# Apokleos/kata-xpu-device-plugin

Measured on NVIDIA H100. Metric: pci.ids parse GB/s (x1000 text + 2^20-key join); device lookups/s reported beside it, higher is better.
Workload: dtype u8

## Files before the change

kata-xpu-device-plugin_b200/csrc/parse_common.cuh:

```cuda
#pragma once
#include "common.cuh"
#include "table.cuh"

namespace kxparse {

constexpr int CW = 2048;
constexpr int HALF = 1024;
constexpr int TRAIL = 16;
constexpr int STG_BYTES = CW + TRAIL;
constexpr int WARPS = 8;
constexpr int NT = WARPS * 32;

constexpr unsigned long long ST_NONE = 1ull << 62;
constexpr unsigned long long ST_PREFIX = 2ull << 62;
constexpr unsigned long long ST_MASK = 3ull << 62;
constexpr unsigned long long CV_HAS_TOP = 1ull << 61;
constexpr unsigned long long CV_VOK = 1ull << 60;
constexpr unsigned long long CV_ANCHOR_MASK = (1ull << 44) - 1;
constexpr uint32_t KX_MAX_PROBE = 1024;
constexpr uint32_t P_NONE = 0xFFFFFFFFu;
#define LS_PUB 0x80000000u
#define LS_TOP 0x40000000u
#define LS_VOK 0x20000000u

__device__ __forceinline__ uint32_t smem_u32(const void *p) { return (uint32_t)__cvta_generic_to_shared(p); }
__device__ __forceinline__ void mbar_init(unsigned long long *bar, uint32_t count) {
    asm volatile("mbarrier.init.shared::cta.b64 [%0], %1;" ::"r"(smem_u32(bar)), "r"(count));
}

__device__ __forceinline__ unsigned long long l2_evict_first_policy() {
    unsigned long long pol;
    asm volatile("createpolicy.fractional.L2::evict_first.b64 %0, 1.0;" : "=l"(pol));
    return pol;
}

__device__ __forceinline__ uint32_t lop3_and_xor(uint32_t a, uint32_t b, uint32_t c) {
    uint32_t d;
    asm("lop3.b32 %0, %1, %2, %3, 0x6A;" : "=r"(d) : "r"(a), "r"(b), "r"(c));
    return d;
}
__device__ __forceinline__ uint32_t lop3_nor_and(uint32_t a, uint32_t b, uint32_t c) {
    uint32_t d;
    asm("lop3.b32 %0, %1, %2, %3, 0x02;" : "=r"(d) : "r"(a), "r"(b), "r"(c));
    return d;
}

__device__ __forceinline__ uint32_t nl_mask16(const uint4 v, uint32_t k7f, uint32_t k0a, uint32_t k80) {
    uint32_t f0 = lop3_nor_and(lop3_and_xor(v.x, k7f, k0a) + k7f, v.x, k80);
    uint32_t f1 = lop3_nor_and(lop3_and_xor(v.y, k7f, k0a) + k7f, v.y, k80);
    uint32_t f2 = lop3_nor_and(lop3_and_xor(v.z, k7f, k0a) + k7f, v.z, k80);
    uint32_t f3 = lop3_nor_and(lop3_and_xor(v.w, k7f, k0a) + k7f, v.w, k80);
    uint32_t lo = __dp4a(f0, 0x08040201u, 0u);
    lo = __dp4a(f1, 0x80402010u, lo);
    uint32_t hi = __dp4a(f2, 0x08040201u, 0u);
    hi = __dp4a(f3, 0x80402010u, hi);
    return (lo >> 7) | (hi << 1);
}

__device__ __forceinline__ bool hex4_swar(uint32_t x, uint32_t &val) {
    uint32_t v = (x & 0x0f0f0f0fu) + ((x >> 6) & 0x01010101u) * 9u;
    uint32_t r = v + 0x30303030u + (((v + 0x06060606u) >> 4) & 0x01010101u) * 0x27u;
    uint32_t s = __byte_perm(v, 0u, 0x0123);
    uint32_t u = s | (s >> 4);
    val = __byte_perm(u, 0u, 0x4420);
    return ((v & 0xf0f0f0f0u) == 0u) & (r == x);
}

__device__ __forceinline__ void table_fold(const KxTableDev &tb, uint32_t key, unsigned long long line_g,
                                           unsigned long long anchor_g, uint32_t &fresh_cnt) {
    uint32_t slot = key == KX_EMPTY_KEY ? tb.cap : (kx_hash(key) >> tb.shift);
    uint4 head = __ldcg(reinterpret_cast<const uint4 *>(&tb.slots[slot]));
    uint32_t k = head.x;
    unsigned long long ml = ((unsigned long long)head.w << 32) | head.z;
    if (key != KX_EMPTY_KEY && k != key) {
        uint32_t step = 0;
        bool fresh = false;
        for (;;) {
            if (k == KX_EMPTY_KEY) {
                uint32_t old = atomicCAS(&tb.slots[slot].key, KX_EMPTY_KEY, key);
                if (old == KX_EMPTY_KEY) {
                    fresh_cnt++;
                    fresh = true;
                    break;
                }
                if (old == key) break;
            }
            slot = (slot + 1) & (tb.cap - 1);
            if (++step >= KX_MAX_PROBE) { tb.counters[KX_C_OVERFLOW] = 1u; return; }
            k = __ldcg(&tb.slots[slot].key);
            if (k == key) break;
        }
        ml = fresh ? KX_NO_OFF : __ldcg(&tb.slots[slot].min_line);
    }
    if (line_g < ml) {
        atomicMin(&tb.slots[slot].min_line, line_g);
        atomicMin(&tb.slots[slot].min_anchor, anchor_g);
    }
}

__device__ __forceinline__ void table_fold_claim2(const KxTableDev &tb, uint32_t key0, unsigned long long line0, unsigned long long anchor0,
                                                  bool on1, uint32_t key1, unsigned long long line1, unsigned long long anchor1,
                                                  uint32_t &fresh_cnt) {
    uint32_t slot0 = key0 == KX_EMPTY_KEY ? tb.cap : (kx_hash(key0) >> tb.shift);
    uint32_t slot1 = key1 == KX_EMPTY_KEY ? tb.cap : (kx_hash(key1) >> tb.shift);
    bool open0 = key0 != KX_EMPTY_KEY, open1 = on1 && key1 != KX_EMPTY_KEY, ok0 = true, ok1 = on1;
    for (uint32_t step = 0; open0 || open1; step++) {
        uint32_t old0 = 0, old1 = 0;
        if (open0) old0 = atomicCAS(&tb.slots[slot0].key, KX_EMPTY_KEY, key0);
        if (open1) old1 = atomicCAS(&tb.slots[slot1].key, KX_EMPTY_KEY, key1);
        if (open0) {
            if (old0 == KX_EMPTY_KEY) { fresh_cnt++; open0 = false; }
            else if (old0 == key0) open0 = false;
            else slot0 = (slot0 + 1) & (tb.cap - 1);
        }
        if (open1) {
            if (old1 == KX_EMPTY_KEY) { fresh_cnt++; open1 = false; }
            else if (old1 == key1) open1 = false;
            else slot1 = (slot1 + 1) & (tb.cap - 1);
        }
        if (step + 1 >= KX_MAX_PROBE && (open0 || open1)) {
            tb.counters[KX_C_OVERFLOW] = 1u;
            ok0 = ok0 && !open0; ok1 = ok1 && !open1;
            break;
        }
    }
    if (ok0) { atomicMin(&tb.slots[slot0].min_line, line0); atomicMin(&tb.slots[slot0].min_anchor, anchor0); }
    if (ok1) { atomicMin(&tb.slots[slot1].min_line, line1); atomicMin(&tb.slots[slot1].min_anchor, anchor1); }
}

__device__ __forceinline__ int32_t table_probe(const KxSlot *__restrict__ slots, uint32_t cap, uint32_t shift, uint32_t key) {
    if (key == KX_EMPTY_KEY) return slots[cap].row;
    uint32_t slot = kx_hash(key) >> shift;
    for (uint32_t step = 0; step < cap; step++) {
        const uint2 kr = __ldg(reinterpret_cast<const uint2 *>(&slots[slot]));
        if (kr.x == key) return (int32_t)kr.y;
        if (kr.x == KX_EMPTY_KEY) return -1;
        slot = (slot + 1) & (cap - 1);
    }
    return -1;
}

__device__ __forceinline__ void table_probe4(const KxSlot *__restrict__ slots, uint32_t cap, uint32_t shift, const uint32_t (&key)[4],
                                             uint32_t on, int32_t (&row)[4]) {
    uint32_t slot[4], open = on & 0xfu;
#pragma unroll
    for (int j = 0; j < 4; j++) {
        row[j] = -1;
        slot[j] = key[j] == KX_EMPTY_KEY ? cap : (kx_hash(key[j]) >> shift);
    }
    for (uint32_t step = 0; open && step < cap; step++) {
        uint2 kr[4];
#pragma unroll
        for (int j = 0; j < 4; j++)
            if ((open >> j) & 1u) kr[j] = __ldg(reinterpret_cast<const uint2 *>(&slots[slot[j]]));
#pragma unroll
        for (int j = 0; j < 4; j++) {
            if (!((open >> j) & 1u)) continue;
            if (slot[j] == cap || kr[j].x == key[j]) { row[j] = (int32_t)kr[j].y; open &= ~(1u << j); }
            else if (kr[j].x == KX_EMPTY_KEY) open &= ~(1u << j);
            else slot[j] = (slot[j] + 1) & (cap - 1);
        }
    }
}

__device__ __forceinline__ uint32_t table_claim(const KxTableDev &tb, uint32_t key, uint32_t &fresh_cnt) {
    if (key == KX_EMPTY_KEY) return tb.cap;
    uint32_t slot = kx_hash(key) >> tb.shift;
    for (uint32_t step = 0; step < KX_MAX_PROBE; step++) {
        const uint32_t k = __ldcg(&tb.slots[slot].key);
        if (k == key) return slot;
        if (k == KX_EMPTY_KEY) {
            const uint32_t old = atomicCAS(&tb.slots[slot].key, KX_EMPTY_KEY, key);
            if (old == KX_EMPTY_KEY) { fresh_cnt++; return slot; }
            if (old == key) return slot;
        }
        slot = (slot + 1) & (tb.cap - 1);
    }
    tb.counters[KX_C_OVERFLOW] = 1u;
    return 0xffffffffu;
}

__device__ __forceinline__ uint32_t table_find(const KxTableDev &tb, uint32_t key) {
    if (key == KX_EMPTY_KEY) return tb.cap;
    uint32_t slot = kx_hash(key) >> tb.shift;
    for (uint32_t step = 0; step < tb.cap; step++) {
        const uint32_t k = __ldg(&tb.slots[slot].key);
        if (k == key) return slot;
        if (k == KX_EMPTY_KEY) return 0xffffffffu;
        slot = (slot + 1) & (tb.cap - 1);
    }
    return 0xffffffffu;
}

__device__ __forceinline__ uint4 lds128(uint32_t a) {
    uint4 v;
    asm volatile("ld.shared.v4.u32 {%0, %1, %2, %3}, [%4];" : "=r"(v.x), "=r"(v.y), "=r"(v.z), "=r"(v.w) : "r"(a));
    return v;
}
__device__ __forceinline__ uint32_t lds32(uint32_t a) {
    uint32_t v;
    asm volatile("ld.shared.u32 %0, [%1];" : "=r"(v) : "r"(a));
    return v;
}
__device__ __forceinline__ uint32_t lds8(uint32_t a) {
    uint32_t v;
    asm volatile("ld.shared.u8 %0, [%1];" : "=r"(v) : "r"(a));
    return v;
}
__device__ __forceinline__ uint32_t lds32_unaligned(uint32_t a) {
    const uint32_t al = a & ~3u;
    return __funnelshift_r(lds32(al), lds32(al + 4u), (a & 3u) * 8u);
}
__device__ __forceinline__ void mbar_expect_tx_a(uint32_t bar, uint32_t bytes) {
    asm volatile("mbarrier.arrive.expect_tx.shared::cta.b64 _, [%0], %1;" ::"r"(bar), "r"(bytes) : "memory");
}
__device__ __forceinline__ bool mbar_try_a(uint32_t bar, uint32_t parity) {
    uint32_t ok;
    asm volatile("{ .reg .pred p; mbarrier.try_wait.parity.shared::cta.b64 p, [%1], %2; selp.u32 %0, 1, 0, p; }"
                 : "=r"(ok)
                 : "r"(bar), "r"(parity)
                 : "memory");
    return ok != 0u;
}
__device__ __forceinline__ void tma_load_a(uint32_t dst, const void *src, uint32_t bytes, uint32_t bar, unsigned long long pol) {
    asm volatile("cp.async.bulk.shared::cluster.global.mbarrier::complete_tx::bytes.L2::cache_hint [%0], [%1], %2, [%3], %4;" ::"r"(dst),
                 "l"(src), "r"(bytes), "r"(bar), "l"(pol)
                 : "memory");
}

__device__ __forceinline__ uint32_t stage_chunk_manual(const uint8_t *text, unsigned long long n, uint32_t g, uint32_t lane,
                                                       uint8_t *dst) {
    const unsigned long long chunk_start = (unsigned long long)g * CW;
    const unsigned long long remain = n - chunk_start;
    const uint32_t n_rel = remain < (unsigned long long)CW ? (uint32_t)remain : (uint32_t)CW + (remain > (unsigned long long)CW);
    for (int cc = (int)lane; cc < STG_BYTES / 16; cc += 32) {
        const unsigned long long q0 = chunk_start + 16ull * (unsigned)cc;
        uint4 v;
        if (q0 + 16 <= n) {
            v = *reinterpret_cast<const uint4 *>(text + q0);
        } else {
            uint8_t tmp[16];
#pragma unroll
            for (int b = 0; b < 16; b++) tmp[b] = q0 + b < n ? text[q0 + b] : (uint8_t)0;
            v = *reinterpret_cast<uint4 *>(tmp);
        }
        *reinterpret_cast<uint4 *>(dst + 16 * cc) = v;
    }
    __syncwarp();
    return n_rel;
}

__device__ __forceinline__ void chunk_masks(uint32_t st, uint32_t lane, uint32_t n_rel, uint32_t k7f, uint32_t k0a, uint32_t k80,
                                            uint32_t (&kh)[2], uint32_t (&th)[2], uint32_t &rawnl) {
    const uint32_t swz = (lane >> 2) & 1u;
    rawnl = 0;
#pragma unroll
    for (int h = 0; h < 2; h++) {
        const uint32_t o = (uint32_t)h * HALF + lane * 32u;
        const uint4 va = lds128(st + o + 16u * swz);
        const uint4 vb = lds128(st + o + 16u * (swz ^ 1u));
        const uint32_t ma = nl_mask16(va, k7f, k0a, k80), mb = nl_mask16(vb, k7f, k0a, k80);
        uint32_t mm = swz ? (mb | (ma << 16)) : (ma | (mb << 16));
        rawnl |= mm;
        if (n_rel <= (uint32_t)CW) mm &= n_rel > o + 1u ? (n_rel - o - 1u >= 32u ? 0xffffffffu : ((1u << (n_rel - o - 1u)) - 1u)) : 0u;
        uint32_t km = 0, tm = 0;
        const uint32_t lp = st + o + 1u;
        while (mm) {
            const uint32_t b = (uint32_t)__ffs((int)mm) - 1u;
            const uint32_t bit = mm & (0u - mm);
            mm ^= bit;
            const uint32_t c0 = lds8(lp + b), c1 = lds8(lp + b + 1u);
            asm("{\n\t.reg .pred p0, pt, pc, pk;\n\t"
                "setp.eq.u32 p0, %2, 9;\n\t"
                "setp.ne.and.u32 pt, %2, 35, !p0;\n\t"
                "setp.ne.and.u32 pc, %3, 9, p0;\n\t"
                "or.pred pk, pt, pc;\n\t"
                "@pt or.b32 %0, %0, %4;\n\t"
                "@pk or.b32 %1, %1, %4;\n\t}"
                : "+r"(tm), "+r"(km)
                : "r"(c0), "r"(c1), "r"(bit));
        }
        kh[h] = km;
        th[h] = tm;
    }
}

__device__ __forceinline__ void fold_lines(const KxTableDev &tab, uint32_t st, unsigned long long cbase, uint32_t m, uint32_t pbase,
                                           uint32_t key_hi, unsigned long long anchor, uint32_t &fresh_cnt) {
    while (m) {
        const uint32_t b = (uint32_t)__ffs((int)m) - 1u;
        m &= m - 1u;
        const uint32_t p = pbase + b;
        uint32_t dv;
        if (hex4_swar(lds32_unaligned(st + p + 1u), dv)) table_fold(tab, key_hi | dv, cbase + p, anchor, fresh_cnt);
    }
}

}

namespace kxparse {
__device__ __forceinline__ void flush_fresh(const KxTableDev &tb, uint32_t &fresh_cnt) {
    const uint32_t tot = __reduce_add_sync(0xffffffffu, fresh_cnt);
    if (tot && (threadIdx.x & 31u) == 0u) atomicAdd(&tb.counters[KX_C_NKEYS], tot);
    fresh_cnt = 0;
}
}
```

kata-xpu-device-plugin_b200/csrc/pciids5.cu:

```cuda
#pragma once
#include "exchange.cuh"
#include "parse_common.cuh"

namespace kxparse5 {

using namespace kxparse;

constexpr int CPC5 = 3;
constexpr int STAGES5 = 2;
constexpr int CTAS5 = 2;
constexpr int COPY5 = CPC5 * CW + TRAIL;
constexpr int RCH5_MAX = CPC5 * STAGES5;
constexpr int RES_WARPS = 8;

struct WarpSmem5 {
    alignas(16) uint8_t stage[STAGES5][COPY5];
    alignas(8) unsigned long long bar[STAGES5];
};

struct Params5 {
    const uint8_t *text;
    unsigned long long n, base;
    uint32_t num_chunks;
    uint32_t tma_limit;
    uint32_t rch;
    uint32_t num_ranges;
    unsigned long long *range_state;
    uint32_t *lead;
    unsigned long long *range_carry;
    uint32_t *tasks;
    KxTableDev tab;
    unsigned long long carry_in;
    uint32_t task_ctas;
    int xa_on;
    uint32_t *xa_done;
    kxx::XaParams xa;
};


__device__ __forceinline__ void nl_masks(uint32_t st, uint32_t lane, uint32_t n_rel, uint32_t k7f, uint32_t k0a, uint32_t k80,
                                         uint32_t (&nl)[2], uint32_t &rawnl) {
    const uint32_t swz = (lane >> 2) & 1u;
    rawnl = 0;
#pragma unroll
    for (int h = 0; h < 2; h++) {
        const uint32_t o = (uint32_t)h * HALF + lane * 32u;
        const uint4 va = lds128(st + o + 16u * swz);
        const uint4 vb = lds128(st + o + 16u * (swz ^ 1u));
        const uint32_t ma = nl_mask16(va, k7f, k0a, k80), mb = nl_mask16(vb, k7f, k0a, k80);
        const uint32_t m2 = ma | (mb << 16);
        uint32_t mm = __funnelshift_l(m2, m2, swz << 4);
        rawnl |= mm;
        if (n_rel <= (uint32_t)CW) mm &= n_rel > o + 1u ? (n_rel - o - 1u >= 32u ? 0xffffffffu : ((1u << (n_rel - o - 1u)) - 1u)) : 0u;
        nl[h] = mm;
    }
}

__device__ __forceinline__ uint32_t tops_of(uint32_t lp, uint32_t mm) {
    uint32_t tm = 0;
    while (mm) {
        const uint32_t bit = mm & (0u - mm);
        mm ^= bit;
        const uint32_t c0 = lds8(lp + (31u - (uint32_t)__clz((int)bit)));
        if (c0 != 9u && c0 != 35u) tm |= bit;
    }
    return tm;
}

__device__ __forceinline__ void tops_of2(uint32_t lp0, uint32_t m0, uint32_t m1, uint32_t &t0, uint32_t &t1) {
    t0 = t1 = 0;
    while (m0 | m1) {
        const uint32_t b0 = m0 & (0u - m0), b1 = m1 & (0u - m1);
        m0 ^= b0;
        m1 ^= b1;
        const uint32_t c0 = lds8(lp0 + (31u - (uint32_t)__clz((int)b0)));
        const uint32_t c1 = lds8(lp0 + (uint32_t)HALF + (31u - (uint32_t)__clz((int)b1)));
        if (c0 != 9u && c0 != 35u) t0 |= b0;
        if (c1 != 9u && c1 != 35u) t1 |= b1;
    }
}

__device__ __forceinline__ uint32_t devs_of(uint32_t lp, uint32_t mm) {
    uint32_t km = 0;
    while (mm) {
        const uint32_t bit = mm & (0u - mm);
        mm ^= bit;
        const uint32_t a = lp + (31u - (uint32_t)__clz((int)bit));
        if (lds8(a) == 9u && lds8(a + 1u) != 9u) km |= bit;
    }
    return km;
}

__global__ void __launch_bounds__(NT, CTAS5) parse_kernel_v5(const Params5 P) {
    extern __shared__ __align__(128) uint8_t smem_raw[];
    WarpSmem5 *W = reinterpret_cast<WarpSmem5 *>(smem_raw);
    uint32_t lane = threadIdx.x & 31u;
    const uint32_t w = threadIdx.x >> 5;
    asm volatile("" : "+r"(lane));
    const uint32_t lt_mask = (1u << lane) - 1u;

    if (lane == 0) {
        for (int s = 0; s < STAGES5; s++) mbar_init(&W[w].bar[s], 1);
        asm volatile("fence.mbarrier_init.release.cluster;" ::: "memory");
    }
    uint32_t tk = 0;
    if (lane == 0) tk = atomicAdd(&P.tab.counters[KX_C_TICKET], 1u);
    uint32_t r = __shfl_sync(0xffffffffu, tk, 0);
    if (r >= P.num_ranges) return;

    uint32_t a_stage0 = smem_u32(smem_raw) + w * (uint32_t)sizeof(WarpSmem5);
    asm volatile("" : "+r"(a_stage0));
    const uint32_t a_bar0 = a_stage0 + (uint32_t)offsetof(WarpSmem5, bar);

    uint32_t k7f = 0x7f7f7f7fu, k0a = 0x0a0a0a0au, k80 = 0x80808080u;
    asm volatile("" : "+r"(k7f), "+r"(k0a), "+r"(k80));

    const unsigned long long pol = l2_evict_first_policy();
    const uint32_t rch = P.rch;
    auto copy_chunks = [](uint32_t cnt, uint32_t k) -> uint32_t {
        return cnt - k * (uint32_t)CPC5 < (uint32_t)CPC5 ? cnt - k * (uint32_t)CPC5 : (uint32_t)CPC5;
    };
    auto issue = [&](uint32_t g0, uint32_t m, uint32_t s) {
        if (g0 + m - 1u < P.tma_limit) {
            mbar_expect_tx_a(a_bar0 + 8u * s, m * (uint32_t)CW + (uint32_t)TRAIL);
            tma_load_a(a_stage0 + s * (uint32_t)COPY5, P.text + (unsigned long long)g0 * CW, m * (uint32_t)CW + (uint32_t)TRAIL, a_bar0 + 8u * s, pol);
        }
    };

    uint32_t phase_bits = 0, s = 0;
    uint32_t nfresh = 0;
    for (;;) {
        uint32_t tk2 = 0;
        if (lane == 0) tk2 = atomicAdd(&P.tab.counters[KX_C_TICKET], 1u);
        uint32_t rc_x = 0, rc_g = 0;
        if (r == 0u) {
            rc_x = LS_PUB | (((P.carry_in & CV_HAS_TOP) && (P.carry_in & CV_VOK)) ? (LS_TOP | LS_VOK) : 0u);
            rc_g = 0xffffffffu;
        }
        uint32_t lead = r == 0u ? 0u : rch;
        const bool table_dead = *reinterpret_cast<volatile uint32_t *>(&P.tab.counters[KX_C_OVERFLOW]) != 0u;
        const uint32_t gb = r * rch;
        const uint32_t cnt = P.num_chunks - gb < rch ? P.num_chunks - gb : rch;
        const uint32_t ncp = (cnt + (uint32_t)CPC5 - 1u) / (uint32_t)CPC5;
        if (lane == 0) {
            for (uint32_t j = 0; j < (uint32_t)STAGES5 && j < ncp; j++) issue(gb + j * (uint32_t)CPC5, copy_chunks(cnt, j), (s + j) % (uint32_t)STAGES5);
        }
        for (uint32_t k = 0; k < ncp; k++) {
            const uint32_t g0 = gb + k * (uint32_t)CPC5, m = copy_chunks(cnt, k);
            const bool by_tma = g0 + m - 1u < P.tma_limit;
            if (by_tma) {
                const uint32_t bar = a_bar0 + 8u * s, par = (phase_bits >> s) & 1u;
                while (!mbar_try_a(bar, par)) {
                }
                phase_bits ^= 1u << s;
            }
            for (uint32_t j = 0; j < m; j++) {
                const uint32_t i = k * (uint32_t)CPC5 + j;
                const uint32_t g = g0 + j;
                const uint32_t st = a_stage0 + s * (uint32_t)COPY5 + j * (uint32_t)CW;
                const unsigned long long cbase = P.base + (unsigned long long)g * CW;
                uint32_t n_rel = CW + 1;
                if (!by_tma) n_rel = stage_chunk_manual(P.text, P.n, g, lane, W[w].stage[s] + j * CW);

                uint32_t nl[2], th[2], rawnl;
                nl_masks(st, lane, n_rel, k7f, k0a, k80, nl, rawnl);
                tops_of2(st + lane * 32u + 1u, nl[0], nl[1], th[0], th[1]);

                uint32_t linfo0 = P_NONE, linfo1 = P_NONE;
                bool any_alive = (g == 0u) || (rc_x & LS_VOK) != 0u;
                {
                    uint32_t t0 = th[0], t1 = th[1];
                    while (t0 | t1) {
                        const bool second = t0 == 0u;
                        const uint32_t tmv = second ? t1 : t0;
                        const uint32_t bit = tmv & (0u - tmv);
                        if (second) t1 = tmv ^ bit; else t0 = tmv ^ bit;
                        const uint32_t p = (second ? (uint32_t)HALF : 0u) + lane * 32u + 1u + (31u - (uint32_t)__clz((int)bit));
                        uint32_t val;
                        const bool ok = hex4_swar(lds32_unaligned(st + p), val);
                        const unsigned long long line_g = cbase + p;
                        bool alive = ok;
                        if (ok) {
                            const unsigned long long vf = P.tab.vendor_first[val];
                            if (line_g < vf) atomicMin(&P.tab.vendor_first[val], line_g);
                            alive = line_g <= vf;
                        }
                        any_alive |= alive;
                        const uint32_t info = (alive ? 0x80000000u : 0u) | ((ok ? val : 0u) << 15) | p;
                        if (second) linfo1 = info; else linfo0 = info;
                    }
                }
                const uint32_t bal0 = __ballot_sync(0xffffffffu, th[0] != 0u);
                const uint32_t bal1 = __ballot_sync(0xffffffffu, th[1] != 0u);
                uint32_t last1;
                if (!__any_sync(0xffffffffu, any_alive)) {
                    const uint32_t bl = bal1 ? bal1 : bal0;
                    last1 = __shfl_sync(0xffffffffu, bal1 ? linfo1 : linfo0, bl ? 31 - __clz((int)bl) : 0);
                    if (bl == 0u) last1 = P_NONE;
                } else {
                    uint32_t kh[2];
                    kh[0] = th[0] | devs_of(st + lane * 32u + 1u, nl[0] & ~th[0]);
                    kh[1] = th[1] | devs_of(st + (uint32_t)HALF + lane * 32u + 1u, nl[1] & ~th[1]);
                    if (table_dead) { kh[0] = th[0]; kh[1] = th[1]; }

                    uint32_t base_info = P_NONE;
                    if (g == 0u && n_rel > 0u) {
                        const uint32_t c0 = lds8(st), c1 = lds8(st + 1u);
                        if (c0 != (uint32_t)'#' && c0 != (uint32_t)'\t') {
                            uint32_t val;
                            const bool ok = hex4_swar(lds32_unaligned(st), val);
                            bool alive = ok;
                            if (ok) {
                                const unsigned long long vf = P.tab.vendor_first[val];
                                if (lane == 0 && cbase < vf) atomicMin(&P.tab.vendor_first[val], cbase);
                                alive = cbase <= vf;
                            }
                            base_info = (alive ? 0x80000000u : 0u) | ((ok ? val : 0u) << 15);
                        } else if (c0 == (uint32_t)'\t' && c1 != (uint32_t)'\t') {
                            uint32_t dv;
                            if (lane == 0 && !table_dead && (P.carry_in & CV_HAS_TOP) && (P.carry_in & CV_VOK) && hex4_swar(lds32_unaligned(st + 1u), dv))
                                table_fold(P.tab, (((uint32_t)(P.carry_in >> 44) & 0xffffu) << 16) | dv, cbase, P.carry_in & CV_ANCHOR_MASK, nfresh);
                        }
                    }
                    linfo0 = linfo1 = P_NONE;
                    {
                        uint32_t t0 = th[0], t1 = th[1];
                        while (t0 | t1) {
                            const bool second = t0 == 0u;
                            const uint32_t tmv = second ? t1 : t0;
                            const uint32_t bit = tmv & (0u - tmv);
                            const uint32_t rest = tmv ^ bit;
                            if (second) t1 = rest; else t0 = rest;
                            const uint32_t pbase = (second ? (uint32_t)HALF : 0u) + lane * 32u + 1u;
                            const uint32_t p = pbase + (31u - (uint32_t)__clz((int)bit));
                            uint32_t val;
                            const bool ok = hex4_swar(lds32_unaligned(st + p), val);
                            const unsigned long long line_g = cbase + p;
                            const bool alive = ok && line_g <= P.tab.vendor_first[val];
                            if (alive) {
                                const uint32_t nxt = rest & (0u - rest);
                                const uint32_t seg = (second ? kh[1] & ~th[1] : kh[0] & ~th[0]) & ~(bit | (bit - 1u)) & (nxt ? nxt - 1u : 0xffffffffu);
                                fold_lines(P.tab, st, cbase, seg, pbase, val << 16, line_g, nfresh);
                            }
                            const uint32_t info = (alive ? 0x80000000u : 0u) | ((ok ? val : 0u) << 15) | p;
                            if (second) linfo1 = info; else linfo0 = info;
                        }
                    }
                    const uint32_t pre0 = kh[0] & ~th[0] & (th[0] ? (th[0] & (0u - th[0])) - 1u : 0xffffffffu);
                    const uint32_t pre1 = kh[1] & ~th[1] & (th[1] ? (th[1] & (0u - th[1])) - 1u : 0xffffffffu);
                    const uint32_t s0 = bal0 & lt_mask, s1 = bal1 & lt_mask;
                    const uint32_t x0 = __shfl_sync(0xffffffffu, linfo0, s0 ? 31 - __clz((int)s0) : 0);
                    const uint32_t l0 = __shfl_sync(0xffffffffu, linfo0, bal0 ? 31 - __clz((int)bal0) : 0);
                    const uint32_t x1 = __shfl_sync(0xffffffffu, linfo1, s1 ? 31 - __clz((int)s1) : 0);
                    const uint32_t l1 = __shfl_sync(0xffffffffu, linfo1, bal1 ? 31 - __clz((int)bal1) : 0);
                    const uint32_t last0 = bal0 ? l0 : base_info;
                    const uint32_t cin0 = s0 ? x0 : base_info;
                    const uint32_t cin1 = s1 ? x1 : last0;
                    last1 = bal1 ? l1 : last0;
                    if (cin0 != P_NONE && (cin0 >> 31))
                        fold_lines(P.tab, st, cbase, pre0, lane * 32u + 1u, ((cin0 >> 15) & 0xffffu) << 16, cbase + (cin0 & 0x7fffu), nfresh);
                    if (cin1 != P_NONE && (cin1 >> 31))
                        fold_lines(P.tab, st, cbase, pre1, (uint32_t)HALF + lane * 32u + 1u, ((cin1 >> 15) & 0xffffu) << 16, cbase + (cin1 & 0x7fffu), nfresh);
                    const uint32_t hw0 = cin0 == P_NONE ? pre0 : 0u;
                    const uint32_t hw1 = cin1 == P_NONE ? pre1 : 0u;
                    if (rc_x & LS_VOK) {
                        uint32_t key_hi = ((rc_x >> 12) & 0xffffu) << 16;
                        unsigned long long anchor = P.base + (unsigned long long)rc_g * CW + (rc_x & 0xfffu);
                        if (rc_g == 0xffffffffu) {
                            key_hi = ((uint32_t)(P.carry_in >> 44) & 0xffffu) << 16;
                            anchor = P.carry_in & CV_ANCHOR_MASK;
                        }
                        if ((hw0 | hw1) != 0u && P.tab.vendor_first[key_hi >> 16] >= anchor) {
                            fold_lines(P.tab, st, cbase, hw0, lane * 32u + 1u, key_hi, anchor, nfresh);
                            fold_lines(P.tab, st, cbase, hw1, (uint32_t)HALF + lane * 32u + 1u, key_hi, anchor, nfresh);
                        }
                    }
                    flush_fresh(P.tab, nfresh);
                }
                if (last1 != P_NONE) {
                    if (rc_x == 0u) lead = i + 1u;
                    rc_x = LS_PUB | LS_TOP | ((last1 >> 31) ? LS_VOK : 0u) | (((last1 >> 15) & 0xffffu) << 12) | (last1 & 0xfffu);
                    rc_g = g;
                }
                if ((bal0 | bal1) == 0u && n_rel > (uint32_t)CW && __reduce_or_sync(0xffffffffu, rawnl) == 0u && lane == 0)
                    atomicOr(&P.tab.counters[KX_C_LONGLINE_HINT], 1u);
                __syncwarp();
            }

            if (lane == 0 && k + (uint32_t)STAGES5 < ncp) issue(gb + (k + (uint32_t)STAGES5) * (uint32_t)CPC5, copy_chunks(cnt, k + (uint32_t)STAGES5), s);
            s = s == (uint32_t)STAGES5 - 1u ? 0u : s + 1u;
        }
        if (lane == 0) {
            unsigned long long v = ST_NONE;
            if (rc_x != 0u) {
                if (rc_g == 0xffffffffu)
                    v = ST_PREFIX | P.carry_in;
                else
                    v = ST_PREFIX | CV_HAS_TOP | ((rc_x & LS_VOK) ? CV_VOK : 0ull) | ((unsigned long long)((rc_x >> 12) & 0xffffu) << 44) |
                        ((P.base + (unsigned long long)rc_g * CW + (rc_x & 0xfffu)) & CV_ANCHOR_MASK);
            }
            P.range_state[r] = v;
            P.lead[r] = lead < cnt ? lead : cnt;
        }
        r = __shfl_sync(0xffffffffu, tk2, 0);
        if (r >= P.num_ranges) break;
    }
}

constexpr uint32_t XA_CTAS = 64;

__global__ void __launch_bounds__(256) resolve_ranges_kernel(const Params5 P) {
    const uint32_t rr = blockIdx.x * blockDim.x + threadIdx.x;
    const uint32_t lane = threadIdx.x & 31u;
    const uint32_t rr0 = rr - lane;
    if (rr0 >= P.num_ranges) return;
    const bool live = rr < P.num_ranges;
    const uint32_t nlead = live ? P.lead[rr] : 0u;
    const unsigned long long own = live ? P.range_state[rr] : ST_NONE;
    const uint32_t pm = __ballot_sync(0xffffffffu, (own & ST_MASK) == ST_PREFIX);
    const uint32_t below = pm & ((1u << lane) - 1u);
    const unsigned long long from_warp = __shfl_sync(0xffffffffu, own, below ? 31 - __clz((int)below) : 0);
    unsigned long long warp_in = 0;
    const uint32_t first_p = pm ? (uint32_t)__ffs((int)pm) - 1u : 32u;
    const bool want = __any_sync(0xffffffffu, nlead != 0u && lane <= first_p);
    if (want) {
        long long q0 = (long long)rr0 - 32;
        for (;;) {
            const long long q = q0 + lane;
            const unsigned long long sv = q >= 0 ? P.range_state[q] : (q == -1 ? (ST_PREFIX | P.carry_in) : ST_NONE);
            const uint32_t m = __ballot_sync(0xffffffffu, (sv & ST_MASK) == ST_PREFIX);
            if (m) {
                warp_in = __shfl_sync(0xffffffffu, sv, 31 - __clz((int)m));
                break;
            }
            q0 -= 32;
        }
    }
    const unsigned long long carry = (below ? from_warp : warp_in) & ~ST_MASK;
    const bool alive = nlead != 0u && (carry & CV_HAS_TOP) && (carry & CV_VOK) &&
                       P.tab.vendor_first[(uint32_t)(carry >> 44) & 0xffffu] >= (carry & CV_ANCHOR_MASK);
    const uint32_t mine = alive ? nlead : 0u;
    uint32_t incl = mine;
#pragma unroll
    for (int d = 1; d < 32; d <<= 1) {
        const uint32_t y = __shfl_up_sync(0xffffffffu, incl, d);
        if (lane >= (uint32_t)d) incl += y;
    }
    const uint32_t tot = __shfl_sync(0xffffffffu, incl, 31);
    uint32_t at0 = 0;
    if (lane == 0 && tot) at0 = atomicAdd(&P.tab.counters[KX_C_DEFER], tot);
    at0 = __shfl_sync(0xffffffffu, at0, 0);
    if (!alive) return;
    P.range_carry[rr] = carry;
    const uint32_t at = at0 + incl - mine;
    for (uint32_t j = 0; j < nlead; j++) P.tasks[at + j] = rr * P.rch + j;
}

__global__ void __launch_bounds__(RES_WARPS * 32) resolve_chunks_kernel(const Params5 P) {
    __shared__ __align__(16) uint8_t stg[RES_WARPS][STG_BYTES];
    __shared__ __align__(8) unsigned long long bars[RES_WARPS];
    __shared__ uint16_t plist[RES_WARPS][704];
    if (blockIdx.x >= P.task_ctas) {
        kxx::xa_push_slice(P.xa, (blockIdx.x - P.task_ctas) * blockDim.x + threadIdx.x, XA_CTAS * blockDim.x);
        __syncthreads();
        if (threadIdx.x == 0) {
            kx_fence_sys();
            const uint32_t prev = atomicAdd(P.xa_done, 1u);
            if (prev == XA_CTAS - 1u) {
                *P.xa_done = 0u;
                kx_fence_sys();
                kxx::xa_finish(P.xa);
            }
        }
        return;
    }
    const uint32_t lane = threadIdx.x & 31u, w = threadIdx.x >> 5;
    const uint32_t lt_mask = (1u << lane) - 1u;
    uint32_t k7f = 0x7f7f7f7fu, k0a = 0x0a0a0a0au, k80 = 0x80808080u;
    asm volatile("" : "+r"(k7f), "+r"(k0a), "+r"(k80));
    const uint32_t st = smem_u32(stg[w]), bar = smem_u32(&bars[w]);
    if (lane == 0) {
        mbar_init(&bars[w], 1);
        asm volatile("fence.mbarrier_init.release.cluster;" ::: "memory");
    }
    __syncwarp();
    const unsigned long long pol = l2_evict_first_policy();
    const uint32_t n_tasks = P.tab.counters[KX_C_DEFER];
    uint32_t par = 0, nfresh = 0;
    const bool small_tab = P.tab.cap <= (1u << 20);
    uint32_t it = 0;
    for (uint32_t t = blockIdx.x * RES_WARPS + w; t < n_tasks; t += P.task_ctas * RES_WARPS, it++) {
        if ((it & 3u) == 0u && *reinterpret_cast<volatile uint32_t *>(&P.tab.counters[KX_C_OVERFLOW]) != 0u) break;
        const uint32_t gg = P.tasks[t];
        uint32_t n_rel = CW + 1;
        if (gg < P.tma_limit) {
            if (lane == 0) {
                mbar_expect_tx_a(bar, STG_BYTES);
                tma_load_a(st, P.text + (unsigned long long)gg * CW, STG_BYTES, bar, pol);
            }
            while (!mbar_try_a(bar, par)) {
            }
            par ^= 1u;
        } else {
            n_rel = stage_chunk_manual(P.text, P.n, gg, lane, stg[w]);
        }
        const unsigned long long cc = P.range_carry[gg / P.rch];
        const uint32_t key_hi = ((uint32_t)(cc >> 44) & 0xffffu) << 16;
        const unsigned long long anchor = cc & CV_ANCHOR_MASK;
        uint32_t kh[2], th[2], rawnl;
        chunk_masks(st, lane, n_rel, k7f, k0a, k80, kh, th, rawnl);
        const uint32_t bal0 = __ballot_sync(0xffffffffu, th[0] != 0u);
        const uint32_t bal1 = __ballot_sync(0xffffffffu, th[1] != 0u);
        const uint32_t pre0 = kh[0] & ~th[0] & (th[0] ? (th[0] & (0u - th[0])) - 1u : 0xffffffffu);
        const uint32_t pre1 = kh[1] & ~th[1] & (th[1] ? (th[1] & (0u - th[1])) - 1u : 0xffffffffu);
        const unsigned long long cbase = P.base + (unsigned long long)gg * CW;
        const uint32_t m0 = (bal0 & lt_mask) == 0u ? pre0 : 0u;
        const uint32_t m1 = (bal0 == 0u && (bal1 & lt_mask) == 0u) ? pre1 : 0u;
        const uint32_t mine = (uint32_t)__popc(m0) + (uint32_t)__popc(m1);
        uint32_t incl = mine;
#pragma unroll
        for (int d = 1; d < 32; d <<= 1) {
            const uint32_t y = __shfl_up_sync(0xffffffffu, incl, d);
            if (lane >= (uint32_t)d) incl += y;
        }
        const uint32_t total = __shfl_sync(0xffffffffu, incl, 31);
        {
            uint32_t idx = incl - mine;
            for (uint32_t m = m0; m; m &= m - 1u) plist[w][idx++] = (uint16_t)(lane * 32u + 1u + (uint32_t)__ffs((int)m) - 1u);
            for (uint32_t m = m1; m; m &= m - 1u) plist[w][idx++] = (uint16_t)((uint32_t)HALF + lane * 32u + 1u + (uint32_t)__ffs((int)m) - 1u);
        }
        __syncwarp();
        if (small_tab) {
            for (uint32_t i = lane; i < total; i += 64u) {
                uint32_t d0, d1 = 0;
                const uint32_t p0 = plist[w][i], p1 = i + 32u < total ? plist[w][i + 32u] : 0u;
                bool v0 = hex4_swar(lds32_unaligned(st + p0 + 1u), d0);
                bool v1 = i + 32u < total && hex4_swar(lds32_unaligned(st + p1 + 1u), d1);
                uint32_t q0 = p0, q1 = p1;
                if (!v0 && v1) { d0 = d1; q0 = p1; v0 = true; v1 = false; }
                if (v0) table_fold_claim2(P.tab, key_hi | d0, cbase + q0, anchor, v1, key_hi | d1, cbase + q1, anchor, nfresh);
            }
        } else {
            for (uint32_t i = lane; i < total; i += 32u) {
                const uint32_t p = plist[w][i];
                uint32_t dv;
                if (hex4_swar(lds32_unaligned(st + p + 1u), dv)) table_fold(P.tab, key_hi | dv, cbase + p, anchor, nfresh);
            }
        }
        __syncwarp();
        flush_fresh(P.tab, nfresh);
    }
}

}
```

Baseline: 2570.

## Replace per-warp TMA bulk staging with register-prefetched vector loads

Drops the mbarrier-driven TMA bulk copies of three-chunk groups. Each chunk is now prefetched one step ahead into registers with 128-bit streaming global loads, plus a cp.async for the trailing bytes, and then stored to shared memory before parsing. Ticket fetching is pipelined across ranges, and the CTA-per-SM bound goes from 2 to 3 because staging needs less shared memory. The cost is more register pressure, extra shared-memory store instructions, and only a single chunk of lookahead instead of two three-chunk TMA stages, so latency hiding may be weaker.

```diff
diff --git a/kata-xpu-device-plugin_b200/csrc/parse_common.cuh b/kata-xpu-device-plugin_b200/csrc/parse_common.cuh
--- a/kata-xpu-device-plugin_b200/csrc/parse_common.cuh
+++ b/kata-xpu-device-plugin_b200/csrc/parse_common.cuh
@@ -206,6 +206,24 @@
     uint32_t v;
     asm volatile("ld.shared.u8 %0, [%1];" : "=r"(v) : "r"(a));
     return v;
+}
+__device__ __forceinline__ void sts128(uint32_t a, const uint4 &v) {
+    asm volatile("st.shared.v4.u32 [%0], {%1, %2, %3, %4};" ::"r"(a), "r"(v.x), "r"(v.y), "r"(v.z), "r"(v.w) : "memory");
+}
+__device__ __forceinline__ uint4 ldg128_stream(const void *p, unsigned long long pol) {
+    uint4 v;
+    asm volatile("ld.global.nc.L2::cache_hint.v4.u32 {%0, %1, %2, %3}, [%4], %5;"
+                 : "=r"(v.x), "=r"(v.y), "=r"(v.z), "=r"(v.w)
+                 : "l"(p), "l"(pol));
+    return v;
+}
+__device__ __forceinline__ void cp_async16(uint32_t dst, const void *src, unsigned long long pol) {
+    asm volatile("cp.async.cg.shared.global.L2::cache_hint [%0], [%1], 16, %2;" ::"r"(dst), "l"(src), "l"(pol) : "memory");
+}
+__device__ __forceinline__ void cp_async_commit() { asm volatile("cp.async.commit_group;" ::: "memory"); }
+template <int N>
+__device__ __forceinline__ void cp_async_wait() {
+    asm volatile("cp.async.wait_group %0;" ::"n"(N) : "memory");
 }
 __device__ __forceinline__ uint32_t lds32_unaligned(uint32_t a) {
     const uint32_t al = a & ~3u;
diff --git a/kata-xpu-device-plugin_b200/csrc/pciids5.cu b/kata-xpu-device-plugin_b200/csrc/pciids5.cu
--- a/kata-xpu-device-plugin_b200/csrc/pciids5.cu
+++ b/kata-xpu-device-plugin_b200/csrc/pciids5.cu
@@ -6,16 +6,20 @@
 
 using namespace kxparse;
 
-constexpr int CPC5 = 3;
-constexpr int STAGES5 = 2;
-constexpr int CTAS5 = 2;
-constexpr int COPY5 = CPC5 * CW + TRAIL;
-constexpr int RCH5_MAX = CPC5 * STAGES5;
+constexpr int AHEAD5 = 1;
+constexpr int STAGES5 = AHEAD5 + 1;
+constexpr int CTAS5 = 3;
+constexpr int RCH5_MAX = 6;
+constexpr int PIECES5 = CW / 16 / 32;
 constexpr int RES_WARPS = 8;
 
 struct WarpSmem5 {
-    alignas(16) uint8_t stage[STAGES5][COPY5];
-    alignas(8) unsigned long long bar[STAGES5];
+    alignas(16) uint8_t stage[STAGES5][STG_BYTES];
+};
+
+struct Ahead5 {
+    uint4 v[PIECES5];
+    uint32_t ri;
 };
 
 struct Params5 {
@@ -99,69 +103,81 @@
     asm volatile("" : "+r"(lane));
     const uint32_t lt_mask = (1u << lane) - 1u;
 
+    uint32_t tk = 0, tk_next = 0;
     if (lane == 0) {
-        for (int s = 0; s < STAGES5; s++) mbar_init(&W[w].bar[s], 1);
-        asm volatile("fence.mbarrier_init.release.cluster;" ::: "memory");
-    }
-    uint32_t tk = 0;
-    if (lane == 0) tk = atomicAdd(&P.tab.counters[KX_C_TICKET], 1u);
-    uint32_t r = __shfl_sync(0xffffffffu, tk, 0);
-    if (r >= P.num_ranges) return;
+        tk = atomicAdd(&P.tab.counters[KX_C_TICKET], 1u);
+        tk_next = atomicAdd(&P.tab.counters[KX_C_TICKET], 1u);
+    }
+    uint32_t pr = __shfl_sync(0xffffffffu, tk, 0), pi = 0;
+    if (pr >= P.num_ranges) return;
 
     uint32_t a_stage0 = smem_u32(smem_raw) + w * (uint32_t)sizeof(WarpSmem5);
     asm volatile("" : "+r"(a_stage0));
-    const uint32_t a_bar0 = a_stage0 + (uint32_t)offsetof(WarpSmem5, bar);
 
     uint32_t k7f = 0x7f7f7f7fu, k0a = 0x0a0a0a0au, k80 = 0x80808080u;
     asm volatile("" : "+r"(k7f), "+r"(k0a), "+r"(k80));
 
     const unsigned long long pol = l2_evict_first_policy();
     const uint32_t rch = P.rch;
-    auto copy_chunks = [](uint32_t cnt, uint32_t k) -> uint32_t {
-        return cnt - k * (uint32_t)CPC5 < (uint32_t)CPC5 ? cnt - k * (uint32_t)CPC5 : (uint32_t)CPC5;
+    uint32_t s_load = 0, s = 0;
+    auto load_ahead = [&](Ahead5 &a) {
+        a.ri = pr << 3 | pi;
+        const uint32_t g = pr * rch + pi;
+        if (pr < P.num_ranges && g < P.tma_limit) {
+            const uint8_t *src = P.text + (unsigned long long)g * CW;
+#pragma unroll
+            for (int j = 0; j < PIECES5; j++) a.v[j] = ldg128_stream(src + 16u * (lane + 32u * j), pol);
+            if (lane == 0) cp_async16(a_stage0 + s_load * (uint32_t)STG_BYTES + (uint32_t)CW, src + CW, pol);
+        }
+        cp_async_commit();
+        s_load = s_load == (uint32_t)STAGES5 - 1u ? 0u : s_load + 1u;
+        if (pr >= P.num_ranges) return;
+        if (++pi == rch || pr * rch + pi == P.num_chunks) {
+            pi = 0;
+            pr = __shfl_sync(0xffffffffu, tk_next, 0);
+            if (lane == 0 && pr < P.num_ranges) tk_next = atomicAdd(&P.tab.counters[KX_C_TICKET], 1u);
+        }
     };
-    auto issue = [&](uint32_t g0, uint32_t m, uint32_t s) {
-        if (g0 + m - 1u < P.tma_limit) {
-            mbar_expect_tx_a(a_bar0 + 8u * s, m * (uint32_t)CW + (uint32_t)TRAIL);
-            tma_load_a(a_stage0 + s * (uint32_t)COPY5, P.text + (unsigned long long)g0 * CW, m * (uint32_t)CW + (uint32_t)TRAIL, a_bar0 + 8u * s, pol);
-        }
-    };
-
-    uint32_t phase_bits = 0, s = 0;
+    Ahead5 q[AHEAD5];
+#pragma unroll
+    for (int a = 0; a < AHEAD5; a++) load_ahead(q[a]);
+
     uint32_t nfresh = 0;
-    for (;;) {
-        uint32_t tk2 = 0;
-        if (lane == 0) tk2 = atomicAdd(&P.tab.counters[KX_C_TICKET], 1u);
-        uint32_t rc_x = 0, rc_g = 0;
-        if (r == 0u) {
-            rc_x = LS_PUB | (((P.carry_in & CV_HAS_TOP) && (P.carry_in & CV_VOK)) ? (LS_TOP | LS_VOK) : 0u);
-            rc_g = 0xffffffffu;
-        }
-        uint32_t lead = r == 0u ? 0u : rch;
-        const bool table_dead = *reinterpret_cast<volatile uint32_t *>(&P.tab.counters[KX_C_OVERFLOW]) != 0u;
-        const uint32_t gb = r * rch;
-        const uint32_t cnt = P.num_chunks - gb < rch ? P.num_chunks - gb : rch;
-        const uint32_t ncp = (cnt + (uint32_t)CPC5 - 1u) / (uint32_t)CPC5;
-        if (lane == 0) {
-            for (uint32_t j = 0; j < (uint32_t)STAGES5 && j < ncp; j++) issue(gb + j * (uint32_t)CPC5, copy_chunks(cnt, j), (s + j) % (uint32_t)STAGES5);
-        }
-        for (uint32_t k = 0; k < ncp; k++) {
-            const uint32_t g0 = gb + k * (uint32_t)CPC5, m = copy_chunks(cnt, k);
-            const bool by_tma = g0 + m - 1u < P.tma_limit;
-            if (by_tma) {
-                const uint32_t bar = a_bar0 + 8u * s, par = (phase_bits >> s) & 1u;
-                while (!mbar_try_a(bar, par)) {
-                }
-                phase_bits ^= 1u << s;
-            }
-            for (uint32_t j = 0; j < m; j++) {
-                const uint32_t i = k * (uint32_t)CPC5 + j;
-                const uint32_t g = g0 + j;
-                const uint32_t st = a_stage0 + s * (uint32_t)COPY5 + j * (uint32_t)CW;
-                const unsigned long long cbase = P.base + (unsigned long long)g * CW;
-                uint32_t n_rel = CW + 1;
-                if (!by_tma) n_rel = stage_chunk_manual(P.text, P.n, g, lane, W[w].stage[s] + j * CW);
-
+    uint32_t rc_x = 0, rc_g = 0;
+    uint32_t lead = 0;
+    bool table_dead = false;
+    uint32_t cnt = 0;
+    while ((q[0].ri >> 3) < P.num_ranges) {
+        const uint32_t r = q[0].ri >> 3, i = q[0].ri & 7u, g = r * rch + i;
+        if (i == 0u) {
+            rc_x = rc_g = 0;
+            if (r == 0u) {
+                rc_x = LS_PUB | (((P.carry_in & CV_HAS_TOP) && (P.carry_in & CV_VOK)) ? (LS_TOP | LS_VOK) : 0u);
+                rc_g = 0xffffffffu;
+            }
+            lead = r == 0u ? 0u : rch;
+            table_dead = *reinterpret_cast<volatile uint32_t *>(&P.tab.counters[KX_C_OVERFLOW]) != 0u;
+            cnt = P.num_chunks - r * rch < rch ? P.num_chunks - r * rch : rch;
+        }
+        {
+            const uint32_t st = a_stage0 + s * (uint32_t)STG_BYTES;
+            const unsigned long long cbase = P.base + (unsigned long long)g * CW;
+            uint32_t n_rel = CW + 1;
+            const bool loaded = g < P.tma_limit;
+            if (loaded) {
+#pragma unroll
+                for (int j = 0; j < PIECES5; j++) sts128(st + 16u * (lane + 32u * j), q[0].v[j]);
+            }
+#pragma unroll
+            for (int a = 0; a + 1 < AHEAD5; a++) q[a] = q[a + 1];
+            load_ahead(q[AHEAD5 - 1]);
+            if (loaded) {
+                cp_async_wait<AHEAD5>();
+                __syncwarp();
+            } else {
+                n_rel = stage_chunk_manual(P.text, P.n, g, lane, W[w].stage[s]);
+            }
+            {
                 uint32_t nl[2], th[2], rawnl;
                 nl_masks(st, lane, n_rel, k7f, k0a, k80, nl, rawnl);
                 tops_of2(st + lane * 32u + 1u, nl[0], nl[1], th[0], th[1]);
@@ -286,10 +302,9 @@
                     atomicOr(&P.tab.counters[KX_C_LONGLINE_HINT], 1u);
                 __syncwarp();
             }
-
-            if (lane == 0 && k + (uint32_t)STAGES5 < ncp) issue(gb + (k + (uint32_t)STAGES5) * (uint32_t)CPC5, copy_chunks(cnt, k + (uint32_t)STAGES5), s);
-            s = s == (uint32_t)STAGES5 - 1u ? 0u : s + 1u;
-        }
+        }
+        s = s == (uint32_t)STAGES5 - 1u ? 0u : s + 1u;
+        if (i + 1u < cnt) continue;
         if (lane == 0) {
             unsigned long long v = ST_NONE;
             if (rc_x != 0u) {
@@ -302,8 +317,6 @@
             P.range_state[r] = v;
             P.lead[r] = lead < cnt ? lead : cnt;
         }
-        r = __shfl_sync(0xffffffffu, tk2, 0);
-        if (r >= P.num_ranges) break;
     }
 }
 
```

Result: no change. 2606 (median of 6 runs) (+1.4%).
